# CliMA/ClimaOcean.jl

Hardware: AMD Instinct MI355X
Metric: flux-kernel surface cells/s (update_state!: JRA55 interp + similarity-theory fluxes + net fluxes) (higher is better)
Workload: dtype f64

## Files before the change

### climaocean.jl_amd/csrc/coflux_lean_kernel.hpp

```cpp
#pragma once
#include <hip/hip_runtime.h>

#include "coflux_halo_device.hpp"
#include "coflux_interp_tiles.hpp"
#include "coflux_lean.hpp"
#include "coflux_certified.hpp"
#include "coflux_solver_shared.hpp"

namespace coflux {

constexpr int LEAN_WAVES = 3;

struct LeanArgs {
    LoopParams L;
    GridDesc G;
    OceanIn O;
    Exchange E;
    FluxOut F;
    const double* g_tab;
    const DevParams* g_params;
    uint32_t* sorted;
    const int* info;
    const int* chunk_begins;
    double z_surface;
    long long mask_kind;
    double T_offset;
    unsigned long long wx_reciprocal;
    long long sort_enabled;
    IceIn I;
    NetOut N;
    SourceDesc S;
    WeightDesc Wt;
    Exchange E_next;
    long long n_chunks;
    long long tail_blocks, tail_rows, tail_cap;
    long long tail_pos;
    HaloRider H;
    long long keep_land;
};
typedef const LeanArgs __attribute__((address_space(4)))* LeanArgsPtr;

hipError_t launch_ao_lean_line(hipStream_t st, bool coare, bool fuse, bool tail, bool halo, int blocks, const LeanArgs& A);

__device__ __forceinline__ LeanArgsPtr opaque(LeanArgsPtr p) {
    asm volatile("" : "+s"(p));
    return p;
}

__device__ __forceinline__ unsigned lean_mix(unsigned idx) { return (idx * 0x9e3779b1u) ^ ((idx * 0x85ebca6bu) >> 15); }
__device__ __forceinline__ unsigned lean_sum(unsigned idx) { return idx * 0xc2b2ae35u + 0x27d4eb2fu; }

constexpr int LEAN_LIST_OFFSET = TABLE_BYTES;
constexpr int LEAN_OFFSET_BITS = 24;
constexpr unsigned LEAN_OFFSET_MASK = (1u << LEAN_OFFSET_BITS) - 1u;
static_assert((long)AO_CHUNK * AO_WET_COST < (1L << LEAN_OFFSET_BITS), "a chunk's range must fit the offset bits");
template <int BLOCK>
struct LeanGeom {
    static_assert(BLOCK == AO_BLOCK, "one workgroup geometry: 256 threads, three workgroups per CU (the 768-thread one-per-CU geometry of rounds 2-5 measured 3 % slower and was retired in round 6)");
    static constexpr int CHUNK = AO_CHUNK;
    static constexpr int WAVES = BLOCK / 64;
    static constexpr int HIST_OFFSET = LEAN_LIST_OFFSET + CHUNK * 4;
    static constexpr int CURSOR_OFFSET = HIST_OFFSET + AO_BINS * 4;
    static constexpr int COUNTERS_OFFSET = CURSOR_OFFSET + AO_BINS * 4;
    static constexpr int WAVEHASH_OFFSET = COUNTERS_OFFSET + 16;
    static constexpr int PARAMS_OFFSET = WAVEHASH_OFFSET + WAVES * 8;
    static constexpr int LDS_BYTES = PARAMS_OFFSET + (int)sizeof(DevParams);
    static_assert(PARAMS_OFFSET % 16 == 0 && LEAN_LIST_OFFSET % 1024 == 0 && (CHUNK * 4) % 1024 == 0, "LDS-DMA pieces");
};
static_assert(LeanGeom<AO_BLOCK>::LDS_BYTES <= 53760, "three narrow lean solver workgroups must fit the CU's 160 KB of LDS");

template <bool FUSE>
__device__ __forceinline__ void lean_zero_cell(const LoopParams& L, double T_offset, const GridDesc& G, LeanArgsPtr K, size_t k, int i, int j) {
    CellFluxes Z{};
    Z.Ts_ocean = -T_offset;
    Z.iterations = L.fixed ? L.maxiter : 0;
    const FluxOut F = kread(&K->F);
    store_fluxes(F, k, Z);
    if constexpr (FUSE) {
        if (i >= 0 && i < G.nx && j >= 0 && j < G.ny) {
            const NetOut N = kread(&K->N);
            store_net_cell(N, k, NetCell{});
        }
    }
}

template <bool COARE, bool FUSE, bool TAIL = false, bool CERT = false, bool LINE = false, bool HALO = false>
__device__ __forceinline__ void ao_lean_body(LeanArgsPtr K_in, int chunk_in) {
    constexpr int BLOCK = AO_BLOCK;
    using Geo = LeanGeom<BLOCK>;
    constexpr int CHUNK = Geo::CHUNK;
    LeanArgsPtr K = opaque(K_in);
    int chunk = chunk_in;
    bool wait_south = false, wait_north = false;
    if constexpr (HALO) {
        static_assert(TAIL && !CERT, "the halo riders belong to the stepping loop's exact-path launch");
        const int nh = K->H.blocks;
        if (chunk < nh) {
            extern __shared__ __attribute__((aligned(16))) char smem_h[];
            const int nf = K->H.F.n, dir = chunk / nf, f = chunk - dir * nf;
            const PeerMailbox M = kread(&K->H.M);
            const GridDesc Gh = kread(&K->G);
            peer_halo_rider(M, K->H.F.ptr[f], f, dir, K->H.rows, K->H.seq, K->H.counters, K->H.expect_sent[dir], K->H.status, Gh, BLOCK,
                            reinterpret_cast<int*>(smem_h));
            return;
        }
        chunk -= nh;
    }
    if constexpr (TAIL) {
        static_assert(BLOCK == 64 * IT_WAVES, "a tail workgroup is an interpolation workgroup");
        const int nb = (int)K->tail_blocks, ipos = (int)K->tail_pos;
        if (chunk >= ipos && chunk < ipos + nb) {
            const SourceDesc S = kread(&K->S);
            const WeightDesc Wt = kread(&K->Wt);
            const GridDesc Gt = kread(&K->G);
            const Exchange En = kread(&K->E_next);
            const int b = chunk - ipos, cap = (int)K->tail_cap, rows = (int)K->tail_rows;
            if (rows == 4) interpolate_tiles<4>(S, Wt, Gt, En, cap, b, nb);
            else if (rows == 2) interpolate_tiles<2>(S, Wt, Gt, En, cap, b, nb);
            else interpolate_tiles<1>(S, Wt, Gt, En, cap, b, nb);
            return;
        }
        if (chunk >= ipos) chunk -= nb;
    }
    if constexpr (HALO) {
        const int cs = K->H.chunk_south, cn = K->H.chunk_north, nc = (int)K->n_chunks;
        if (K->H.blocks > 0) {
            if (cs <= cn) {
                const int inner = cn - cs;
                chunk = chunk < inner ? cs + chunk : (chunk - inner < cs ? chunk - inner : cn + (chunk - inner - cs));
            }
            wait_south = K->H.wait_south != 0 && chunk < cs;
            wait_north = K->H.wait_north != 0 && chunk >= cn && chunk < nc;
        }
    }
    const LoopParams L = kread(&K->L);
    const GridDesc G = kread(&K->G);
    const double* __restrict__ g_tab = K->g_tab;
    const DevParams* __restrict__ g_params = K->g_params;
    const void* mask = K->O.mask;
    extern __shared__ __attribute__((aligned(16))) char smem[];
    double* tab = reinterpret_cast<double*>(smem);
    unsigned* list = reinterpret_cast<unsigned*>(smem + LEAN_LIST_OFFSET);
    int* hist = reinterpret_cast<int*>(smem + Geo::HIST_OFFSET);
    int* cursor = reinterpret_cast<int*>(smem + Geo::CURSOR_OFFSET);
    int* counters = reinterpret_cast<int*>(smem + Geo::COUNTERS_OFFSET);
    unsigned* wavehash = reinterpret_cast<unsigned*>(smem + Geo::WAVEHASH_OFFSET);
    DevParams* lp = reinterpret_cast<DevParams*>(smem + Geo::PARAMS_OFFSET);
    const int tid = threadIdx.x, lane = tid & 63, wave = tid >> 6;
    const int wx = G.nx + 2 * G.ring;
    const unsigned wx_rcp = (unsigned)K->wx_reciprocal;
    const bool use_static = K->sorted != nullptr;
    static_assert(sizeof(DevParams) % 16 == 0 && sizeof(DevParams) <= 1024, "the parameter block is one LDS-DMA piece");
    if (tid < (int)(sizeof(DevParams) / 16))
        __builtin_amdgcn_global_load_lds((const __attribute__((address_space(1))) void*)(reinterpret_cast<const char*>(g_params) + lane * 16),
                                         (__attribute__((address_space(3))) void*)(smem + Geo::PARAMS_OFFSET), 16, 0, 0);
    static_assert(TABLE_BYTES % 1024 == 0, "the table stage copies whole 1 KB pieces");
    {
        const char* gb = reinterpret_cast<const char*>(g_tab);
        constexpr int PIECES = TABLE_BYTES / 1024, WAVES = Geo::WAVES;
#pragma unroll
        for (int r = 0; r < (PIECES + WAVES - 1) / WAVES; ++r) {
            const int c = wave + r * WAVES;
            if (c < PIECES)
                __builtin_amdgcn_global_load_lds((const __attribute__((address_space(1))) void*)(gb + c * 1024 + lane * 16),
                                                 (__attribute__((address_space(3))) void*)(smem + c * 1024), 16, 0, 0);
        }
    }
    if (use_static) {
        const char* gl = reinterpret_cast<const char*>(K->sorted + (size_t)chunk * CHUNK);
        constexpr int PIECES = CHUNK * 4 / 1024, WAVES = Geo::WAVES;
#pragma unroll
        for (int r = 0; r < (PIECES + WAVES - 1) / WAVES; ++r) {
            const int c = wave + r * WAVES;
            if (c < PIECES)
                __builtin_amdgcn_global_load_lds((const __attribute__((address_space(1))) void*)(gl + c * 1024 + lane * 16),
                                                 (__attribute__((address_space(3))) void*)(smem + LEAN_LIST_OFFSET + c * 1024), 16, 0, 0);
        }
    }
    constexpr int LAND_UNROLL = 8;
    typedef const __attribute__((address_space(1))) unsigned* GlobalWords;
    unsigned raw_lo[LAND_UNROLL], raw_hi[LAND_UNROLL], raw_shift = 0;
    const __attribute__((address_space(4))) int* cb = (const __attribute__((address_space(4))) int*)K->chunk_begins;
    const int range_begin = cb[chunk], range_end = cb[chunk + 1];
    int listed = 0;
    unsigned want_x = 0, want_y = 0;
    if (use_static) {
        const __attribute__((address_space(4))) int* ci = (const __attribute__((address_space(4))) int*)K->info;
        listed = ci[chunk * 4];
        want_x = (unsigned)ci[chunk * 4 + 1];
        want_y = (unsigned)ci[chunk * 4 + 2];
    }
    const int mask_kind = (mask == nullptr) ? CF_MASK_NONE : (int)K->mask_kind;
    const double z_surface = K->z_surface;
    const double T_offset = K->T_offset;
    const bool keep_land = K->keep_land != 0;
    const bool sorting = !CERT && use_static && K->sort_enabled != 0;
    const int sort_windows = (int)K->sort_enabled;
    float inv_window = 0.f;
    auto lean_bin = [&](int q, int trips) -> int {
        if (sort_windows <= 1) return AO_BINS - 1 - trip_bin(trips);
        const int w = min((int)(((float)q + 0.5f) * inv_window), sort_windows - 1);
        const int bpw = AO_BINS / sort_windows, lo = bpw >= 16 ? 5 : 8;
        return w * bpw + (bpw - 1 - min(max(trips - lo, 0), bpw - 1));
    };
    {
        const unsigned long long mbase = mask_kind == CF_MASK_NONE ? (unsigned long long)g_tab : (unsigned long long)mask;
        const unsigned stride = mask_kind == CF_MASK_NONE ? 0u : (mask_kind == CF_MASK_U8 ? 1u : 8u);
        const unsigned hi_step = mask_kind == CF_MASK_BOTTOM_HEIGHT ? 4u : 0u;
#pragma unroll
        for (int n = 0; n < LAND_UNROLL; ++n) {
            const int ic = min(range_begin + tid + n * BLOCK, range_end - 1);
            const int jj = row_of(ic, wx, wx_rcp);
            const unsigned long long a = mbase + (unsigned long long)cell_index(G, ic - jj * wx - G.ring, jj - G.ring) * stride;
            raw_shift |= ((unsigned)a & 3u) << (2 * n);
            raw_lo[n] = *(GlobalWords)(a & ~3ull);
            raw_hi[n] = *(GlobalWords)((a & ~3ull) + hi_step);
        }
    }
    if (tid < 4) counters[tid] = 0;
    if (tid < AO_BINS) hist[tid] = 0;
    if constexpr (CERT) {
        if (tid < 2 * AO_BINS) hist[tid] = -1;
    }
    __builtin_amdgcn_s_waitcnt(0x0f70);
#pragma unroll
    for (int n = 0; n < LAND_UNROLL; ++n) asm volatile("" : "+v"(raw_lo[n]), "+v"(raw_hi[n]));
    unsigned hx = 0, hy = 0, land = 0;
#pragma unroll
    for (int n = 0; n < LAND_UNROLL; ++n) {
        const int idx = range_begin + tid + n * BLOCK;
        const bool w = mask_kind == CF_MASK_NONE ? true
                       : mask_kind == CF_MASK_U8 ? ((raw_lo[n] >> (8 * ((raw_shift >> (2 * n)) & 3u))) & 0xffu) != 0
                                                 : !(z_surface <= __hiloint2double((int)raw_hi[n], (int)raw_lo[n]));
        if (idx < range_end) {
            if (w) {
                hx ^= lean_mix((unsigned)idx);
                hy += lean_sum((unsigned)idx);
            } else {
                land |= 1u << n;
            }
        }
    }
    for (int idx = range_begin + tid + LAND_UNROLL * BLOCK; idx < range_end; idx += BLOCK) {
        const int jj = row_of(idx, wx, wx_rcp);
        const size_t k = cell_index(G, idx - jj * wx - G.ring, jj - G.ring);
        const bool w = mask_kind == CF_MASK_NONE ? true
                       : mask_kind == CF_MASK_U8 ? ((const uint8_t*)mask)[k] != 0 : !(z_surface <= ((const double*)mask)[k]);
        if (w) {
            hx ^= lean_mix((unsigned)idx);
            hy += lean_sum((unsigned)idx);
        } else if (!keep_land) {
            lean_zero_cell<FUSE>(L, T_offset, G, opaque(K), k, idx - jj * wx - G.ring, jj - G.ring);
        }
    }
    for (int d = 32; d; d >>= 1) {
        hx ^= (unsigned)__shfl_xor((int)hx, d);
        hy += (unsigned)__shfl_xor((int)hy, d);
    }
    if (lane == 0) {
        wavehash[2 * wave] = hx;
        wavehash[2 * wave + 1] = hy;
    }
    __syncthreads();
    if constexpr (HALO) {
        if (wait_south) peer_halo_wait(&opaque(K)->H.counters[2], K->H.expect_done[0]);
        if (wait_north) peer_halo_wait(&opaque(K)->H.counters[3], K->H.expect_done[1]);
    }
    const DevParams& P = *lp;
    bool have_list = false;
    int nwet = 0;
    if (use_static) {
        unsigned got_x = 0, got_y = 0;
#pragma unroll
        for (int w = 0; w < Geo::WAVES; ++w) {
            got_x ^= wavehash[2 * w];
            got_y += wavehash[2 * w + 1];
        }
        have_list = got_x == want_x && got_y == want_y;
        nwet = listed;
        if (sort_windows > 1 && nwet > 0)
            inv_window = 1.0f / (float)(((nwet + sort_windows * 64 - 1) / (sort_windows * 64)) * 64);
    }
    if (have_list && land && !keep_land) {
        LeanArgsPtr Kz = opaque(K);
#pragma unroll
        for (int n = 0; n < LAND_UNROLL; ++n)
            if (land & (1u << n)) {
                const int idx = range_begin + tid + n * BLOCK;
                const int jj = row_of(idx, wx, wx_rcp);
                const int i = idx - jj * wx - G.ring, j = jj - G.ring;
                lean_zero_cell<FUSE>(L, T_offset, G, Kz, cell_index(G, i, j), i, j);
            }
    }
    int begin = range_begin, end = range_end;
    for (;;) {
        if (!have_list) {
            for (int base = begin; base < end; base += BLOCK) {
                const int idx = base + tid;
                bool wet = false;
                if (idx < end) {
                    const int jj = row_of(idx, wx, wx_rcp);
                    const int i = idx - jj * wx - G.ring, j = jj - G.ring;
                    const size_t k = cell_index(G, i, j);
                    wet = cell_is_wet(P, mask, k);
                    if (!wet) lean_zero_cell<FUSE>(L, T_offset, G, opaque(K), k, i, j);
                }
                const unsigned long long m = __ballot(wet);
                int wave_base = 0;
                if (lane == 0 && m) wave_base = atomicAdd(&counters[2], __popcll(m));
                wave_base = __shfl(wave_base, 0);
                if (wet) {
                    const int p = wave_base + __popcll(m & ((1ull << lane) - 1ull));
                    if (p < CHUNK) list[p] = (unsigned)(idx - range_begin);
                }
            }
            __syncthreads();
            nwet = counters[2];
            if (nwet > CHUNK) {
                end = begin + CHUNK;
                __syncthreads();
                if (tid < 4) counters[tid] = 0;
                if constexpr (CERT) {
                    if (tid < 2 * AO_BINS) hist[tid] = -1;
                }
                __syncthreads();
                continue;
            }
        }
        auto store_result = [&](double* base, unsigned byte_off, double v) {
            if constexpr (FUSE) gstore_final(base, byte_off, v);
            else gstore(base, byte_off, v);
        };
        auto claim = [&]() {
            int st = 0;
            if (lane == 0) st = atomicAdd(&counters[0], 64);
            return __shfl(st, 0);
        };
        constexpr int QUEUE_CAP = 2 * AO_BINS;
        constexpr int QUEUE_CLOSED = 1 << 20;
        int* queue = hist;
        static_assert(Geo::CURSOR_OFFSET == Geo::HIST_OFFSET + AO_BINS * 4, "the exact-path queue spans the histogram and the cursors");
        bool straggling = false;
        int limit = nwet;
        auto position_of = [&](int st) -> int {
            const int qq = min(st + lane, limit - 1);
            if constexpr (CERT) return straggling ? queue[qq] : qq;
            return qq;
        };
        auto coords_of = [&](int st, int& ci, int& cj) -> size_t {
            const int idx = range_begin + (int)(list[position_of(st)] & LEAN_OFFSET_MASK);
            const int jj = row_of(idx, wx, wx_rcp);
            ci = idx - jj * wx - G.ring;
            cj = jj - G.ring;
            return cell_index(G, ci, cj);
        };
        auto cell_of = [&](int st) -> size_t {
            int ci, cj;
            return coords_of(st, ci, cj);
        };
        struct Raw {
            double ua, va, Ta, pa, qa, u0, u1, v0, v1, To, So;
        };
        auto request = [&](int st) {
            int ci, cj;
            const size_t k = coords_of(st, ci, cj);
            LeanArgsPtr Kb = opaque(K);
            const double* __restrict__ Ou = Kb->O.u;
            const double* __restrict__ Ov = Kb->O.v;
            const unsigned k8 = (unsigned)k * 8u;
            Raw r;
            r.u0 = gload(Ou, k8);
            r.u1 = gload(Ou, k8 + 8u);
            r.v0 = gload(Ov, k8);
            r.v1 = gload(Ov, k8 + (unsigned)G.sj * 8u);
            r.To = gload(Kb->O.T, k8);
            r.So = gload(Kb->O.S, k8);
            r.ua = gload(Kb->E.u, k8);
            r.va = gload(Kb->E.v, k8);
            r.Ta = gload(Kb->E.T, k8);
            r.pa = gload(Kb->E.p, k8);
            r.qa = gload(Kb->E.q, k8);
            return r;
        };
        int start = claim();
        Raw raw{};
        if (start < nwet) raw = request(start);
        for (;;) {
            if constexpr (CERT) {
                if (!straggling && start >= nwet) {
                    int filled = 0;
                    if (lane == 0) filled = atomicAdd(&counters[1], QUEUE_CLOSED);
                    filled = __shfl(filled, 0);
                    if (filled <= 0 || filled >= QUEUE_CLOSED) break;
                    limit = min(filled, QUEUE_CAP);
                    for (int e = lane; e < limit; e += 64)
                        while (__hip_atomic_load(&queue[e], __ATOMIC_ACQUIRE, __HIP_MEMORY_SCOPE_WORKGROUP) < 0) __builtin_amdgcn_s_sleep(1);
                    straggling = true;
                    start = 0;
                    raw = request(start);
                }
            }
            if (start >= limit) break;
            const int q = start + lane;
            const bool in_range = q < limit;
            double Mp_now = 0.0;
            const double raw_So = raw.So;
            if constexpr (CERT) {
                if (!straggling) Mp_now = gload(opaque(K)->E.Mp, (unsigned)cell_of(start) * 8u);
            }
            const LeanCell c = lean_prologue(P, L.kappa, tab, raw.ua, raw.va, raw.Ta, raw.pa, raw.qa, 0.5 * (raw.u0 + raw.u1),
                                             0.5 * (raw.v0 + raw.v1), raw.To, raw.So);
            if (in_range) store_result(opaque(K)->F.Ts, (unsigned)cell_of(start) * 8u, c.Ts - T_offset);
            CertNetSalt net_salt;
            if constexpr (CERT) {
                net_salt.Mp = (float)Mp_now;
                net_salt.floor_v = CERT_JS_FLOOR * __builtin_amdgcn_rcpf((float)raw_So * (float)P.rho_f_inv);
            }
            Scales s;
            bool finish = in_range;
            if constexpr (CERT) {
                bool exact = in_range;
                if (!straggling) {
                    const LoopParams Lc = kread(&opaque(K)->L);
                    s = mo_iterate_certified<COARE>(Lc, c, tab, in_range, exact, net_salt);
                    const unsigned long long m = __builtin_amdgcn_ballot_w64(exact);
                    const bool in_place = ((volatile int*)counters)[1] == 0 && ((volatile int*)counters)[0] >= nwet;
                    if (m && !in_place) {
                        int slot = 0;
                        if (lane == 0) slot = atomicAdd(&counters[1], __popcll(m));
                        slot = __shfl(slot, 0) + __popcll(m & ((1ull << lane) - 1ull));
                        if (exact && slot < QUEUE_CAP) {
                            __hip_atomic_store(&queue[slot], q, __ATOMIC_RELEASE, __HIP_MEMORY_SCOPE_WORKGROUP);
                            exact = false;
                            finish = false;
                        }
                    }
                }
                if (__builtin_amdgcn_ballot_w64(exact) != 0ull) {
                    const LoopParams Le = kread(&opaque(K)->L);
                    const Scales e = mo_iterate_lean<COARE, false>(Le, c, tab, exact);
                    if (exact) {
                        s = e;
                        s.it |= CERT_EXACT_FLAG;
                    }
                }
            } else {
                if constexpr (LINE) s = mo_iterate_lean_line<COARE>(L, c, tab, in_range);
                else s = mo_iterate_lean<COARE>(L, c, tab, in_range);
            }
            if (finish) {
                LeanArgsPtr Ke = opaque(K);
                const size_t k = cell_of(start);
                const CellFluxes R = lean_epilogue(c, T_offset, s);
                const FluxOut F = kread(&Ke->F);
                const unsigned k8 = (unsigned)k * 8u;
                store_result(F.Qc, k8, R.Qc);
                store_result(F.Qv, k8, R.Qv);
                store_result(F.Fv, k8, R.Fv);
                gstore(F.tx, k8, R.rho_tau_x);
                gstore(F.ty, k8, R.rho_tau_y);
                if (F.ustar) gstore_final(F.ustar, k8, R.ustar);
                if (F.tstar) gstore_final(F.tstar, k8, R.tstar);
                if (F.qstar) gstore_final(F.qstar, k8, R.qstar);
                if (F.iters) gstore_i32(F.iters, (unsigned)k * 4u, R.iterations);
                if constexpr (FUSE) {
                    const int idx = range_begin + (int)(list[position_of(start)] & LEAN_OFFSET_MASK);
                    const int jj = row_of(idx, wx, wx_rcp);
                    const int ci = idx - jj * wx - G.ring, cj = jj - G.ring;
                    if (ci >= 0 && ci < G.nx && cj >= 0 && cj < G.ny) {
                        const IceIn I = kread(&Ke->I);
                        const NetOut N = kread(&Ke->N);
                        const double Ts_ocean = (gload(Ke->O.T, k8) + P.T_offset) - T_offset;
                        const NetCell C = net_cell_local(P, P.albedo, I.conc ? gload(I.conc, k8) : 0.0, gload(Ke->O.S, k8), Ts_ocean + P.T_offset,
                                                         gload(Ke->E.Mp, k8), gload(Ke->E.Qs, k8), gload(Ke->E.Ql, k8), R.Qc, R.Qv, R.Fv,
                                                         I.Qio ? gload(I.Qio, k8) : 0.0, I.Jsio ? gload(I.Jsio, k8) : 0.0,
                                                         I.land ? gload(I.land, k8) : 0.0);
                        gstore_final(N.T, k8, C.JT);
                        gstore_final(N.S, k8, C.JS);
                        if (N.sw) gstore_final(N.sw, k8, C.sw);
                        if (N.lw_up) gstore_final(N.lw_up, k8, C.lw_up);
                        if (N.lw_down) gstore_final(N.lw_down, k8, C.lw_down);
                        if (N.sw_down) gstore_final(N.sw_down, k8, C.sw_down);
                    }
                }
                if (sorting && have_list) {
                    const int w = min(s.work, 255);
                    list[q] = (list[q] & LEAN_OFFSET_MASK) | ((unsigned)w << LEAN_OFFSET_BITS);
                    atomicAdd(&hist[lean_bin(q, w)], 1);
                }
            }
            int next;
            if constexpr (CERT) next = straggling ? start + 64 : claim();
            else next = claim();
            if (next < limit) raw = request(next);
            start = next;
        }
        if (have_list || end >= range_end) break;
        begin = end;
        end = range_end;
        __syncthreads();
        if (tid < 4) counters[tid] = 0;
        if constexpr (CERT) {
            if (tid < 2 * AO_BINS) hist[tid] = -1;
        }
        __syncthreads();
    }
    if (sorting && have_list) {
        __syncthreads();
        if (tid < AO_BINS) {
            const int v = hist[tid];
            int incl = v;
#pragma unroll
            for (int d = 1; d < 64; d <<= 1) {
                const int up = __shfl_up(incl, d);
                if (lane >= d) incl += up;
            }
            cursor[tid] = incl - v;
        }
        __syncthreads();
        uint32_t* out = opaque(K)->sorted + (size_t)chunk * CHUNK;
        constexpr int PER_THREAD = CHUNK / BLOCK;
        unsigned word[PER_THREAD];
        int at[PER_THREAD];
#pragma unroll
        for (int n = 0; n < PER_THREAD; ++n) word[n] = list[min(tid + n * BLOCK, CHUNK - 1)];
#pragma unroll
        for (int n = 0; n < PER_THREAD; ++n)
            at[n] = tid + n * BLOCK < nwet ? atomicAdd(&cursor[lean_bin(tid + n * BLOCK, (int)(word[n] >> LEAN_OFFSET_BITS))], 1) : -1;
#pragma unroll
        for (int n = 0; n < PER_THREAD; ++n)
            if (at[n] >= 0) out[at[n]] = word[n] & LEAN_OFFSET_MASK;
    }
}

}
```

### climaocean.jl_amd/csrc/coflux_solver.hip

```cpp
#include <hip/hip_runtime.h>

#include <cstring>

#include "coflux_solver_shared.hpp"
#include "coflux_lean.hpp"
#include "coflux_lean_kernel.hpp"

namespace coflux {

int wet_list_stride();
struct Geom {
    static constexpr int CHUNK = AO_CHUNK;
    static constexpr int COUNTERS_OFFSET = TABLE_DOUBLES * 8 + CHUNK * 4;
    static constexpr int PARAMS_OFFSET = COUNTERS_OFFSET + 16 + 2 * 64 * 4;
    static constexpr int LDS_BYTES = PARAMS_OFFSET + (int)sizeof(DevParams);
};
constexpr int AO_LAYER_1 = AO_CHUNK < 1024 ? AO_CHUNK : 1024, AO_LAYER_2 = AO_CHUNK < 768 ? AO_CHUNK : 768, AO_LAYER_3 = 512;
static_assert(AO_LAYER_1 <= AO_CHUNK && AO_LAYER_1 >= AO_LAYER_2 && AO_LAYER_2 >= AO_LAYER_3, "layer sizes");
static_assert(AO_BINS == 64, "Geom::PARAMS_OFFSET spells the bin count out");
static_assert(Geom::LDS_BYTES <= 53760, "three narrow solver workgroups must fit the CU's 160 KB of LDS");


constexpr int AO_MAX_ROUNDS = 8;
struct ChunkRounds {
// ... 411 lines not shown
            } else if (!keep_land) {
                SolverArgsPtr Kz = opaque(K);
                const FluxOut F = kread(&Kz->F);
                const NetOut N = kread(&Kz->N);
                zero_cell<FUSE_NET>(L, T_offset, G, F, N, k, i, j);
                        if constexpr (seaice_spec(SPEC)) ice_zero_net(opaque(K), G, k, i, j);
            }
        }
        for (int d = 32; d; d >>= 1) {
            hx ^= (unsigned)__shfl_xor((int)hx, d);
            hy ^= (unsigned)__shfl_xor((int)hy, d);
        }
        if (lane == 0) {
            atomicXor(reinterpret_cast<unsigned*>(&counters[2]), hx);
            atomicXor(reinterpret_cast<unsigned*>(&counters[3]), hy);
        }
        if (!unsorted) {
            __syncthreads();
            if (tid < 64) {
                const int v = lane < AO_BINS ? hist[lane] : 0;
                int incl = v;
#pragma unroll
                for (int d = 1; d < 64; d <<= 1) {
                    const int up = __shfl_up(incl, d);
                    if (lane >= d) incl += up;
                }
                if (lane < AO_BINS) bin_start[lane] = incl - v;
                if (lane == 63) counters[0] = incl;
            }
            __syncthreads();
#pragma unroll
            for (int n = 0; n < PER_THREAD; ++n)
                if (my_idx[n] >= 0) {
                    const int p = atomicAdd(&bin_start[AO_BINS - 1 - trip_bin(my_trip[n])], 1);
                    list[p] = ((unsigned)(tid + n * BLOCK) << AO_LIST_OFFSET_BITS) | (unsigned)(my_idx[n] - range_begin);
                }
        }
        __builtin_amdgcn_s_waitcnt(0x0f70);
        __syncthreads();
        nwet = counters[0];
        have_list = (counters[2] | counters[3]) == 0;
        if (have_list) {
            if (land && !keep_land) {
                SolverArgsPtr Kz = opaque(K);
                const FluxOut F = kread(&Kz->F);
                const NetOut N = kread(&Kz->N);
#pragma unroll
                for (int n = 0; n < LAND_UNROLL; ++n)
                    if (land & (1u << n)) {
                        const int idx = range_begin + tid + n * BLOCK;
                        const int jj = row_of(idx, wx, wx_rcp);
                        const int i = idx - jj * wx - G.ring, j = jj - G.ring;
                        zero_cell<FUSE_NET>(L, T_offset, G, F, N, cell_index(G, i, j), i, j);
                        if constexpr (seaice_spec(SPEC)) ice_zero_net(opaque(K), G, cell_index(G, i, j), i, j);
                    }
            }
        } else {
            use_static = false;
            __syncthreads();
            if (tid < 4) counters[tid] = 0;
            __syncthreads();
        }
    }
    if (!use_static) {
        __builtin_amdgcn_s_waitcnt(0x0f70);
        __syncthreads();
    }
    int begin = range_begin, end = range_end;
    for (;;) {
        if (!have_list) {
            for (int base = begin; base < end; base += BLOCK) {
                const int idx = base + tid;
                bool wet = false;
                if (idx < end) {
                    const int jj = row_of(idx, wx, wx_rcp);
                    const int i = idx - jj * wx - G.ring, j = jj - G.ring;
                    const size_t k = cell_index(G, i, j);
                    wet = cell_is_wet(P, mask, k);
                    if (!wet) {
                        SolverArgsPtr Kz = opaque(K);
                        const FluxOut F = kread(&Kz->F);
                        const NetOut N = kread(&Kz->N);
                        zero_cell<FUSE_NET>(L, T_offset, G, F, N, k, i, j);
                        if constexpr (seaice_spec(SPEC)) ice_zero_net(opaque(K), G, k, i, j);
                    }
                }
                const unsigned long long m = __ballot(wet);
                int wave_base = 0;
                if (lane == 0 && m) wave_base = atomicAdd(&counters[0], __popcll(m));
                wave_base = __shfl(wave_base, 0);
                if (wet) {
                    const int p = wave_base + __popcll(m & ((1ull << lane) - 1ull));
                    if (p < CHUNK) list[p] = (unsigned)(idx - range_begin);
                }
            }
            __builtin_amdgcn_s_waitcnt(0x0f70);
            __syncthreads();
            nwet = counters[0];
            if (nwet > CHUNK) {
                end = begin + CHUNK;
                __syncthreads();
                if (tid < 4) counters[tid] = 0;
                __syncthreads();
                continue;
            }
        }
        for (;;) {
            int start = 0;
            if (lane == 0) start = atomicAdd(&counters[1], 64);
            start = __shfl(start, 0);
            if (start >= nwet) break;
            const int q = start + lane;
            const bool in_range = q < nwet;
            const int qc = in_range ? q : nwet - 1;
            if constexpr (seaice_spec(SPEC)) {
                const IceParams Ice = kread(&K->Ice);
                IceConsts c;
                double Ts;
                bool ice_free = false;
                {
                    const int idx = range_begin + (int)(list[qc] & ((1u << AO_LIST_OFFSET_BITS) - 1u));
                    const int jj = row_of(idx, wx, wx_rcp);
                    const size_t k = cell_index(G, idx - jj * wx - G.ring, jj - G.ring);
                    SolverArgsPtr Kb = opaque(K);
                    const IceStateIn S = kread(&Kb->S);
                    const double ua = Kb->E.u[k], va = Kb->E.v[k], Ta = Kb->E.T[k], pa = Kb->E.p[k], qa = Kb->E.q[k];
                    const double inv_Ta = frcp(Ta);
                    const double lam_a = liquid_fraction_fast(P, logt, Ta);
                    const AirState A = air_state_fast(P, pa, Ta, inv_Ta, qa, lam_a, svp_equil_fast(P, logt, Ta, inv_Ta, lam_a));
                    c.rho = A.rho;
                    c.cp = A.cp_m;
                    c.qav = A.q_vap;
                    c.Ls = P.LH_s0 + (P.cp_v - P.cp_i) * (Ta - P.T_0);
                    c.Ti = Ice.T_fw - Ice.liquidus_slope * Kb->O.S[k];
                    c.hk = fmax(S.thickness[k] * Ice.inv_k, Ice.hk_min);
                    const double alb = S.albedo ? S.albedo[k] : Ice.albedo;
                    c.Qd = -(1.0 - alb) * Kb->E.Qs[k] - Ice.emissivity * Kb->E.Ql[k];
                    c.theta_a = Ta + P.g * P.h_ref * frcp(A.cp_m);
                    c.pa = pa;
                    c.du = ua;
                    c.dv = va;
                    if (P.velocity_difference == CF_VELOCITY_RELATIVE) {
                        c.du = ua - (S.u ? S.u[k] : 0.0);
                        c.dv = va - (S.v ? S.v[k] : 0.0);
                    }
                    c.dU2 = c.du * c.du + c.dv * c.dv;
                    c.dU = fsqrt(c.dU2);
                    c.dU2 = __builtin_fma(c.dU2, P.wind2_scale, P.wind2_add);
                    double alpha = P.rm.charnock;
                    if (P.rm.kind == CF_ROUGHNESS_WIND_CHARNOCK)
                        alpha = fmax(P.rm.charnock, P.rm.wind_a1 * fmin(c.dU, P.rm.wind_umax) + P.rm.wind_a2);
                    c.alpha_g = alpha * P.inv_g;
                    Ts = S.top_temperature[k] + Ice.T_offset;
                    if (Ice.ice_free_zero != 0.0 && S.concentration) ice_free = S.concentration[k] == 0.0 && S.thickness[k] == 0.0;
                }
                Scales s{0.0, 0.0, 0.0, 0, 0};
                const bool solve = in_range && !ice_free;
                if (__ballot(solve) != 0ull) {
                    bool left = false, unused = false;
                    if constexpr (seaice_lean_spec(SPEC)) {
                        const LeanIceConsts lc{c.rho, c.cp, c.qav, c.Ls, c.Ti, c.hk, c.Qd, c.theta_a, c.pa, frcp1(c.pa), frcp1(c.rho * P.R_v), c.dU2};
                        s = ice_iterate_lean<COARE, seaice_lin_spec(SPEC)>(P, L, Ice, lc, tab, solve, Ts, left);
                        if (__ballot(left) != 0ull) {
                            double Ts2 = ice_carried_skin(opaque(K), G, range_begin, list[qc], wx, wx_rcp) + Ice.T_offset;
                            const Scales s2 = ice_iterate_lean<COARE, seaice_lin_spec(SPEC), true>(P, L, Ice, lc, tab, left, Ts2, unused);
                            if (left) { s = s2; Ts = Ts2; }
                        }
                    } else {
                        s = ice_iterate<COARE, seaice_lin_spec(SPEC)>(P, L, Ice, c, tab, solve, Ts, left);
                        if (__ballot(left) != 0ull) {
                            double Ts2 = ice_carried_skin(opaque(K), G, range_begin, list[qc], wx, wx_rcp) + Ice.T_offset;
                            const Scales s2 = ice_iterate<COARE, seaice_lin_spec(SPEC), true>(P, L, Ice, c, tab, left, Ts2, unused);
                            if (left) { s = s2; Ts = Ts2; }
                        }
                    }
                }
                if (ice_free) s = Scales{0.0, 0.0, 0.0, 0, 0};
                if (in_range) {
                    SolverArgsPtr Ke = opaque(K);
                    const int idx2 = range_begin + (int)(list[qc] & ((1u << AO_LIST_OFFSET_BITS) - 1u));
                    const int jj2 = row_of(idx2, wx, wx_rcp);
                    const size_t k = cell_index(G, idx2 - jj2 * wx - G.ring, jj2 - G.ring);
                    CellFluxes R;
                    const double inv_dU = (c.dU == 0.0) ? 0.0 : frcp(c.dU);
                    const double tau = -s.us * s.us * inv_dU;
                    const double rho_u = c.rho * s.us;
                    R.Fv = -rho_u * s.qq;
                    R.Qv = R.Fv * c.Ls;
                    R.Qc = -rho_u * c.cp * s.ts;
                    R.rho_tau_x = c.rho * tau * c.du;
                    R.rho_tau_y = c.rho * tau * c.dv;
                    R.Ts_ocean = Ts - Ice.T_offset;
                    if (ice_free) R.Ts_ocean = kread(&Ke->S).top_temperature[k];
                    R.ustar = s.us;
                    R.tstar = s.ts;
                    R.qstar = s.qq;
                    R.iterations = s.it;
                    const FluxOut F = kread(&Ke->F);
                    store_fluxes(F, k, R);
                    {
                        const NetIceOut NI = kread(&Ke->NI);
                        const int ci = idx2 - jj2 * wx - G.ring, cj = jj2 - G.ring;
                        if (NI.top && ci >= 0 && ci < G.nx && cj >= 0 && cj < G.ny) {
                            const IceStateIn S2 = kread(&Ke->S);
                            double top, bottom;
                            net_sea_ice_cell(S2.albedo ? S2.albedo[k] : Ice.albedo, Ice.emissivity, Ice.eps_sigma, Ice.T_offset, Ke->E.Qs[k],
                                             Ke->E.Ql[k], R.Ts_ocean, R.Qc, R.Qv, NI.conc[k], NI.frazil ? NI.frazil[k] : 0.0,
                                             NI.interface_heat ? NI.interface_heat[k] : 0.0, top, bottom);
                            NI.top[k] = top;
                            NI.bottom[k] = bottom;
                        }
                    }
                    if (use_static && W.trip) store_hint(&W.trip[(size_t)chunk * CHUNK + (list[qc] >> AO_LIST_OFFSET_BITS)], s.work);
                }
                continue;
            }
            static_assert(SPEC != SOLVER_OCEAN_LEAN, "the ocean presets run in coflux_solver_lean.hip");
            CellConsts c;
            double So;
            {
                const int idx = range_begin + (int)(list[qc] & ((1u << AO_LIST_OFFSET_BITS) - 1u));
                const int jj = row_of(idx, wx, wx_rcp);
                const size_t k = cell_index(G, idx - jj * wx - G.ring, jj - G.ring);
                SolverArgsPtr Kb = opaque(K);
            const double* __restrict__ Ou = Kb->O.u;
            const double* __restrict__ Ov = Kb->O.v;
            const double uo = 0.5 * (Ou[k] + Ou[k + 1]);
            const double vo = 0.5 * (Ov[k] + Ov[k + (size_t)G.sj]);
                So = Kb->O.S[k];
                c = cell_prologue(P, L.min_gust, logt, Kb->E.u[k], Kb->E.v[k], Kb->E.T[k], Kb->E.p[k], Kb->E.q[k], uo, vo,
                                  Kb->O.T[k], So);
            }
            Scales s;
            if constexpr (SPEC == SOLVER_LY)
                s = ly_iterate(L, c, tab);
            else
                s = mo_iterate<COARE, SPEC>(L, c, tab, in_range);
            if (in_range) {
                SolverArgsPtr Ke = opaque(K);
                const int idx2 = range_begin + (int)(list[qc] & ((1u << AO_LIST_OFFSET_BITS) - 1u));
                const int jj2 = row_of(idx2, wx, wx_rcp);
                const int ci = idx2 - jj2 * wx - G.ring, cj = jj2 - G.ring;
                const size_t k = cell_index(G, ci, cj);
                const CellFluxes R = cell_epilogue(c, P.T_offset, s);
                {
                    const FluxOut F = kread(&Ke->F);
                    store_fluxes<FUSE_NET>(F, k, R);
                }
                if (use_static && W.trip) W.trip[(size_t)chunk * CHUNK + (list[qc] >> AO_LIST_OFFSET_BITS)] = (uint8_t)min(s.work, 255);
                if constexpr (FUSE_NET) {
                    if (ci >= 0 && ci < G.nx && cj >= 0 && cj < G.ny) {
                        const IceIn I = kread(&Ke->I);
                        const NetOut N = kread(&Ke->N);
                        store_net_cell<true>(N, k, net_cell_local(P, P.albedo, I.conc ? I.conc[k] : 0.0, So, R.Ts_ocean + P.T_offset,
                                                            Ke->E.Mp[k], Ke->E.Qs[k], Ke->E.Ql[k], R.Qc, R.Qv, R.Fv,
                                                            I.Qio ? I.Qio[k] : 0.0, I.Jsio ? I.Jsio[k] : 0.0, I.land ? I.land[k] : 0.0));
                    }
                }
            }
        }
        if (use_static || end >= range_end) break;
        begin = end;
        end = range_end;
        __syncthreads();
        if (tid < 4) counters[tid] = 0;
        __syncthreads();
    }
}

template <bool COARE, int SPEC, bool FUSE_NET, bool TAIL = false>
__global__ __launch_bounds__(AO_BLOCK, 3) void ao_flux_fast_kernel(SolverArgs unused_by_name) {
    ao_flux_fast_body<COARE, SPEC, FUSE_NET, TAIL>((SolverArgsPtr)__builtin_amdgcn_kernarg_segment_ptr(), (int)blockIdx.x);
}

struct IceOceanArgs {
    SolverArgs A;
    LeanArgs O;
    long long ocean_chunks;
    int nseg, seg_kind[8], seg_first[8], seg_count[8];
};
template <bool COARE_ICE, bool COARE_OCEAN, int ICE_SPEC>
__global__ __launch_bounds__(AO_BLOCK, 3) void ice_ocean_kernel(IceOceanArgs unused_by_name) {
    typedef const IceOceanArgs __attribute__((address_space(4)))* ArgsPtr;
    ArgsPtr K = (ArgsPtr)__builtin_amdgcn_kernarg_segment_ptr();
    asm volatile("" : "+s"(K));
    int block = (int)blockIdx.x;
    const int nch = (int)K->A.n_chunks, noc = (int)K->ocean_chunks;
    (void)noc;
    int kind = 0, idx = 0;
    {
        int rest = block;
        const int ns = K->nseg;
        for (int q = 0; q < ns; ++q) {
            const int c = K->seg_count[q];
            if (rest < c) {
                kind = K->seg_kind[q];
                idx = K->seg_first[q] + rest;
                break;
            }
            rest -= c;
        }
    }
    if (kind == 1) {
        ao_lean_body<COARE_OCEAN, true>((LeanArgsPtr)&K->O, idx);
        return;
    }
    block = kind == 2 ? nch + idx : idx;
    ao_flux_fast_body<COARE_ICE, ICE_SPEC, false, true>((SolverArgsPtr)&K->A, block);
}

__global__ void debug_eval_kernel(int fn, int n, const double* __restrict__ x, double* __restrict__ y,
                                  const double* __restrict__ g_tab) {
    extern __shared__ __attribute__((aligned(16))) char smem[];
    double* tab = reinterpret_cast<double*>(smem);
    stage_tables(tab, g_tab, threadIdx.x, blockDim.x);
    __syncthreads();
    const double* logt = tab + LOG_OFFSET;
    for (int k = blockIdx.x * blockDim.x + threadIdx.x; k < n; k += gridDim.x * blockDim.x) {
        const double v = x[k];
        double r;
        switch (fn) {
            case 0: r = flog(logt, v); break;
            case 1: r = fexp(v); break;
            case 2: r = fcbrt(v); break;
            case 3: r = fsqrt(v); break;
            case 4: r = frcp(v); break;
            case 5: r = psi_eval(tab, 0, psi_arg(v)); break;
            case 6: r = psi_eval(tab, 1, psi_arg(v)); break;
            case 7: r = __builtin_amdgcn_rcp(v); break;
            case 8: r = __builtin_amdgcn_rsq(v); break;
            case 9: {
                double q = __builtin_amdgcn_rcp(v);
                r = __builtin_fma(q, __builtin_fma(-v, q, 1.0), q);
            } break;
            default: r = 0.0;
        }
        y[k] = r;
    }
}


template <bool COARE, bool FUSE>
static void launch_ao_spec(hipStream_t st, dim3 grid, const LaunchCfg& L, const LoopParams& C, const GridDesc& G,
                           const OceanIn& O, const Exchange& E, const FluxOut& F, const IceIn& I, const NetOut& N,
                           double z_surface, long long mask_kind, double T_offset) {
    SolverArgs A{C, G, O, E, F, L.d_tables, L.d_params, WetLists{L.d_wet_pos, C.specialization == SOLVER_LY ? nullptr : L.d_trip},
                 L.d_chunk_begins, I, N, IceStateIn{}, IceParams{},
                 z_surface, mask_kind, T_offset, row_reciprocal(G.nx + 2 * G.ring)};
    A.keep_land = L.keep_land;
#define CF_LAUNCH(COARE_, SPEC_) \
    hipLaunchKernelGGL((ao_flux_fast_kernel<COARE_, SPEC_, FUSE>), grid, dim3(AO_BLOCK), Geom::LDS_BYTES, st, A)
    switch (C.specialization) {
        case SOLVER_ICE: CF_LAUNCH(COARE, SOLVER_ICE); break;
        case SOLVER_LY: CF_LAUNCH(true, SOLVER_LY); break;
        default: CF_LAUNCH(COARE, SOLVER_GENERIC);
    }
#undef CF_LAUNCH
}

hipError_t launch_ly_fluxes_with_tail(hipStream_t st, const LaunchCfg& L, const DevParams& P, const LoopParams& C, const GridDesc& G,
                                      const cf_ocean_surface* o, const cf_exchange_fields* e, const cf_interface_fluxes* f,
                                      const cf_sea_ice_fields* ice, const cf_net_ocean_fluxes* net, const double* land,
                                      const cf_atmos_source* next_src, const cf_interp_weights* w, const cf_exchange_fields* next_out,
                                      int tail_rows, int tail_blocks) {
    if (!L.d_chunk_begins || L.n_chunks <= 0 || !net || !next_src || !w || !next_out || L.interp_cap <= 0 || tail_blocks <= 0 ||
        C.specialization != SOLVER_LY)
        return hipErrorInvalidValue;
    if ((size_t)IT_WAVES * CF_JRA55_NVARS * L.interp_cap * sizeof(double) > (size_t)Geom::LDS_BYTES) return hipErrorInvalidValue;
    const IceIn I = make_ice_in(ice, land);
    const NetOut N = make_net_out(net);
    SolverArgs A{C, G, make_ocean(o), make_exchange(e), make_fluxes(f), L.d_tables, L.d_params, WetLists{L.d_wet_pos, nullptr},
                 L.d_chunk_begins, I, N, IceStateIn{}, IceParams{}, P.z_surface, P.mask_kind, P.T_offset, row_reciprocal(G.nx + 2 * G.ring)};
    A.Si = make_source(next_src);
    A.Wi = make_weights(w);
    A.E_next = make_exchange(next_out);
    A.n_chunks = L.n_chunks;
    A.tail_blocks = tail_blocks;
    A.tail_rows = tail_rows;
    A.tail_cap = L.interp_cap;
    A.keep_land = L.keep_land;
    hipLaunchKernelGGL((ao_flux_fast_kernel<true, SOLVER_LY, true, true>), dim3(L.n_chunks + tail_blocks), dim3(AO_BLOCK),
                       Geom::LDS_BYTES, st, A);
    return hipGetLastError();
}

hipError_t launch_ao_fluxes(hipStream_t st, const LaunchCfg& L, const DevParams& P, const LoopParams& C,
                            const GridDesc& G, const cf_ocean_surface* o, const cf_exchange_fields* e,
                            const cf_interface_fluxes* f, const cf_sea_ice_fields* ice, const cf_net_ocean_fluxes* net,
                            const double* land) {
    if (L.solver == CF_SOLVER_LIBM) return net ? hipErrorInvalidValue : launch_ao_fluxes_libm(st, P, G, o, e, f);
    if (C.specialization == SOLVER_OCEAN_LEAN) {
        if (!L.d_lean_info) return hipErrorInvalidValue;
        return launch_ao_fluxes_lean(st, L, P, C, G, o, e, f, ice, net, land);
    }
    OceanIn O = make_ocean(o);
    Exchange E = make_exchange(e);
    FluxOut F = make_fluxes(f);
    const IceIn I = make_ice_in(ice, land);
    const NetOut N = make_net_out(net);
    if (!L.d_chunk_begins || L.n_chunks <= 0) return hipErrorInvalidValue;
    dim3 grid(L.n_chunks);
    const bool coare = P.similarity_form == CF_SIMILARITY_COARE_LOGARITHMIC;
    if (net) {
        if (coare) launch_ao_spec<true, true>(st, grid, L, C, G, O, E, F, I, N, P.z_surface, P.mask_kind, P.T_offset);
        else launch_ao_spec<false, true>(st, grid, L, C, G, O, E, F, I, N, P.z_surface, P.mask_kind, P.T_offset);
    } else {
        if (coare) launch_ao_spec<true, false>(st, grid, L, C, G, O, E, F, I, N, P.z_surface, P.mask_kind, P.T_offset);
        else launch_ao_spec<false, false>(st, grid, L, C, G, O, E, F, I, N, P.z_surface, P.mask_kind, P.T_offset);
    }
    return hipGetLastError();
}

hipError_t launch_ai_fluxes(hipStream_t st, const LaunchCfg& L, const DevParams& P, const LoopParams& C, const IceParams& Ice,
                            const GridDesc& G, const cf_sea_ice_state* ice, const cf_ocean_surface* o,
                            const cf_exchange_fields* e, const cf_interface_fluxes* f, const double* d_tables,
                            const DevParams* d_params, uint8_t* d_trip, const AiTail* tail, const NetIceOut* net_ice) {
    if (!L.d_chunk_begins || L.n_chunks <= 0) return hipErrorInvalidValue;
    SolverArgs A{};
    A.L = C;
    A.G = G;
    A.O = make_ocean(o);
    A.E = make_exchange(e);
    A.F = make_fluxes(f);
    A.g_tab = d_tables;
    A.g_params = d_params;
    A.W = WetLists{L.d_wet_pos, d_trip};
    A.chunk_begins = L.d_chunk_begins;
    A.S = IceStateIn{ice->thickness, ice->top_temperature, ice->u, ice->v, ice->albedo, Ice.ice_free_zero != 0.0 ? ice->concentration : nullptr};
    A.Ice = Ice;
    A.z_surface = P.z_surface;
    A.mask_kind = P.mask_kind;
    A.T_offset = P.T_offset;
    A.wx_reciprocal = row_reciprocal(G.nx + 2 * G.ring);
    dim3 grid(L.n_chunks);
    const bool coare = P.similarity_form == CF_SIMILARITY_COARE_LOGARITHMIC;
    const bool lean = C.specialization == SOLVER_ICE && L.solver == CF_SOLVER_TABLES;
    const bool lin = Ice.skin_scheme == CF_SKIN_LINEARISED;
    if (net_ice) A.NI = *net_ice;
    if (tail) {
        if (!lean) return hipErrorInvalidValue;
        A.n_chunks = L.n_chunks;
        if (tail->next_out) {
            if (!tail->next_src || !tail->w || L.interp_cap <= 0 || tail->interp_blocks <= 0 ||
                (size_t)IT_WAVES * CF_JRA55_NVARS * L.interp_cap * sizeof(double) > (size_t)Geom::LDS_BYTES)
                return hipErrorInvalidValue;
            A.Si = make_source(tail->next_src);
            A.Wi = make_weights(tail->w);
            A.E_next = make_exchange(tail->next_out);
            A.tail_blocks = tail->interp_blocks;
            A.tail_rows = tail->interp_rows;
            A.tail_cap = L.interp_cap;
        }
        if (tail->stress_net) {
            if (!tail->d_ocean_params || !tail->stress_ocean || !tail->stress_fluxes) return hipErrorInvalidValue;
            A.stress_blocks = (G.nx * G.ny + 255) / 256;
            A.stress_params = tail->d_ocean_params;
            A.stress_mask = tail->stress_ocean->mask;
            A.rtx = tail->stress_fluxes->x_momentum;
            A.rty = tail->stress_fluxes->y_momentum;
            A.stress_ice = make_ice_in(tail->stress_ice, nullptr);
            A.tau_x = tail->stress_net->u;
            A.tau_y = tail->stress_net->v;
        }
        if (tail->ocean) {
            if (!tail->ocean->valid || tail->stress_net || tail->ocean->n_chunks <= 0) return hipErrorInvalidValue;
            static_assert(sizeof(LeanArgs) <= sizeof(tail->ocean->args), "OceanRider::args holds a LeanArgs");
            IceOceanArgs M{};
            M.A = A;
            memcpy(&M.O, tail->ocean->args, sizeof(LeanArgs));
            M.ocean_chunks = tail->ocean->n_chunks;
            {
                const int noc_all = tail->ocean->n_chunks, head = std::min(std::max(L.cu_count, 0), noc_all);
                M.seg_kind[0] = 1; M.seg_first[0] = 0; M.seg_count[0] = head;
                M.seg_kind[1] = 0; M.seg_first[1] = 0; M.seg_count[1] = L.n_chunks;
                M.seg_kind[2] = 1; M.seg_first[2] = head; M.seg_count[2] = noc_all - head;
                M.seg_kind[3] = 2; M.seg_first[3] = 0; M.seg_count[3] = (int)A.tail_blocks;
                M.nseg = 4;
            }
            const dim3 mgrid((unsigned)(L.n_chunks + tail->ocean->n_chunks + A.tail_blocks));
            constexpr size_t lds = (size_t)(Geom::LDS_BYTES > LeanGeom<AO_BLOCK>::LDS_BYTES ? Geom::LDS_BYTES : LeanGeom<AO_BLOCK>::LDS_BYTES);
            static_assert(lds <= 53760, "three workgroups per CU");
#define CF_IO_LAUNCH(SPEC_)                                                                                                   \
    do {                                                                                                                      \
        if (coare) {                                                                                                          \
            if (tail->ocean->coare) hipLaunchKernelGGL((ice_ocean_kernel<true, true, SPEC_>), mgrid, dim3(AO_BLOCK), lds, st, M); \
            else hipLaunchKernelGGL((ice_ocean_kernel<true, false, SPEC_>), mgrid, dim3(AO_BLOCK), lds, st, M);              \
        } else {                                                                                                              \
            if (tail->ocean->coare) hipLaunchKernelGGL((ice_ocean_kernel<false, true, SPEC_>), mgrid, dim3(AO_BLOCK), lds, st, M); \
            else hipLaunchKernelGGL((ice_ocean_kernel<false, false, SPEC_>), mgrid, dim3(AO_BLOCK), lds, st, M);             \
        }                                                                                                                     \
    } while (0)
            if (lin) CF_IO_LAUNCH(SOLVER_SEAICE_LEAN_LIN);
            else CF_IO_LAUNCH(SOLVER_SEAICE_LEAN);
#undef CF_IO_LAUNCH
            return hipGetLastError();
        }
        const dim3 tgrid((unsigned)(L.n_chunks + A.tail_blocks + A.stress_blocks));
#define CF_AI_TAIL_LAUNCH(COARE_, SPEC_) \
    hipLaunchKernelGGL((ao_flux_fast_kernel<COARE_, SPEC_, false, true>), tgrid, dim3(AO_BLOCK), Geom::LDS_BYTES, st, A)
        if (lin) { if (coare) CF_AI_TAIL_LAUNCH(true, SOLVER_SEAICE_LEAN_LIN); else CF_AI_TAIL_LAUNCH(false, SOLVER_SEAICE_LEAN_LIN); }
        else { if (coare) CF_AI_TAIL_LAUNCH(true, SOLVER_SEAICE_LEAN); else CF_AI_TAIL_LAUNCH(false, SOLVER_SEAICE_LEAN); }
#undef CF_AI_TAIL_LAUNCH
        return hipGetLastError();
    }
#define CF_AI_LAUNCH(COARE_, SPEC_) \
    hipLaunchKernelGGL((ao_flux_fast_kernel<COARE_, SPEC_, false>), grid, dim3(AO_BLOCK), Geom::LDS_BYTES, st, A)
    if (lin) {
        if (lean) { if (coare) CF_AI_LAUNCH(true, SOLVER_SEAICE_LEAN_LIN); else CF_AI_LAUNCH(false, SOLVER_SEAICE_LEAN_LIN); }
        else { if (coare) CF_AI_LAUNCH(true, SOLVER_SEAICE_LIN); else CF_AI_LAUNCH(false, SOLVER_SEAICE_LIN); }
    } else {
        if (lean) { if (coare) CF_AI_LAUNCH(true, SOLVER_SEAICE_LEAN); else CF_AI_LAUNCH(false, SOLVER_SEAICE_LEAN); }
        else { if (coare) CF_AI_LAUNCH(true, SOLVER_SEAICE); else CF_AI_LAUNCH(false, SOLVER_SEAICE); }
    }
#undef CF_AI_LAUNCH
    return hipGetLastError();
}

extern "C" int cf_debug_chunk_plan(long long total_cost, int cu_count, int forced_wet_per_chunk, int* out, int capacity) {
    ChunkRounds R{};
    plan_chunk_rounds((long)total_cost, cu_count, forced_wet_per_chunk, &R);
    if (!out || capacity < 1 + 2 * R.n) return -1;
    out[0] = R.n;
    for (int r = 0; r < R.n; ++r) {
        out[1 + 2 * r] = R.cost[r] / AO_WET_COST;
        const long span = (long)R.base[r + 1] - R.base[r];
        out[2 + 2 * r] = (int)((span + R.cost[r] - 1) / R.cost[r]);
    }
    return AO_WET_COST;
}

hipError_t launch_debug_eval(hipStream_t st, const LaunchCfg& L, int fn, int n, const double* x, double* y) {
    hipLaunchKernelGGL(debug_eval_kernel, dim3(64), dim3(256), TABLE_BYTES, st, fn, n, x, y, L.d_tables);
    return hipGetLastError();
}

}
```

Measured before the change: 10.23 billion.

## Software-pipeline lean solver: prefetch next cell and its prologue across the epilogue

In the non-certified lean path, the next cell's claim and input loads are issued before the current cell's epilogue and stores. The next cell's prologue is computed ahead of the loop body. The net-flux inputs for the current cell are also loaded early, and the coordinates come from coords_of instead of a list lookup. The aim is to hide global-memory latency behind epilogue and store work, at the cost of more live registers. The combined ocean/ice kernel explicitly opts out of this path.

Result: faster. 10.38 billion, median of 6 (+1.5%).

```diff
diff --git a/climaocean.jl_amd/csrc/coflux_lean_kernel.hpp b/climaocean.jl_amd/csrc/coflux_lean_kernel.hpp
--- a/climaocean.jl_amd/csrc/coflux_lean_kernel.hpp
+++ b/climaocean.jl_amd/csrc/coflux_lean_kernel.hpp
@@ -84,7 +84,7 @@
     }
 }
 
-template <bool COARE, bool FUSE, bool TAIL = false, bool CERT = false, bool LINE = false, bool HALO = false>
+template <bool COARE, bool FUSE, bool TAIL = false, bool CERT = false, bool LINE = false, bool HALO = false, bool BURST_BOUNDARY = true>
 __device__ __forceinline__ void ao_lean_body(LeanArgsPtr K_in, int chunk_in) {
     constexpr int BLOCK = AO_BLOCK;
     using Geo = LeanGeom<BLOCK>;
@@ -327,6 +327,7 @@
                 continue;
             }
         }
+        constexpr bool BURST = BURST_BOUNDARY && !CERT;
         auto store_result = [&](double* base, unsigned byte_off, double v) {
             if constexpr (FUSE) gstore_final(base, byte_off, v);
             else gstore(base, byte_off, v);
@@ -385,6 +386,10 @@
         int start = claim();
         Raw raw{};
         if (start < nwet) raw = request(start);
+        LeanCell ahead{};
+        if constexpr (BURST) {
+            if (start < nwet) ahead = lean_prologue(P, L.kappa, tab, raw.ua, raw.va, raw.Ta, raw.pa, raw.qa, 0.5 * (raw.u0 + raw.u1), 0.5 * (raw.v0 + raw.v1), raw.To, raw.So);
+        }
         for (;;) {
             if constexpr (CERT) {
                 if (!straggling && start >= nwet) {
@@ -408,8 +413,9 @@
             if constexpr (CERT) {
                 if (!straggling) Mp_now = gload(opaque(K)->E.Mp, (unsigned)cell_of(start) * 8u);
             }
-            const LeanCell c = lean_prologue(P, L.kappa, tab, raw.ua, raw.va, raw.Ta, raw.pa, raw.qa, 0.5 * (raw.u0 + raw.u1),
-                                             0.5 * (raw.v0 + raw.v1), raw.To, raw.So);
+            LeanCell c;
+            if constexpr (BURST) c = ahead;
+            else c = lean_prologue(P, L.kappa, tab, raw.ua, raw.va, raw.Ta, raw.pa, raw.qa, 0.5 * (raw.u0 + raw.u1), 0.5 * (raw.v0 + raw.v1), raw.To, raw.So);
             if (in_range) store_result(opaque(K)->F.Ts, (unsigned)cell_of(start) * 8u, c.Ts - T_offset);
             CertNetSalt net_salt;
             if constexpr (CERT) {
@@ -448,52 +454,125 @@
                 if constexpr (LINE) s = mo_iterate_lean_line<COARE>(L, c, tab, in_range);
                 else s = mo_iterate_lean<COARE>(L, c, tab, in_range);
             }
-            if (finish) {
-                LeanArgsPtr Ke = opaque(K);
-                const size_t k = cell_of(start);
+            if constexpr (BURST) {
+                struct NetRaw {
+                    double To, So, Mp, Qs, Ql, conc, Qio, Jsio, land;
+                };
+                auto request_net = [&](unsigned k8) {
+                    LeanArgsPtr Ke = opaque(K);
+                    NetRaw n;
+                    n.To = gload(Ke->O.T, k8);
+                    n.So = gload(Ke->O.S, k8);
+                    n.Mp = gload(Ke->E.Mp, k8);
+                    n.Qs = gload(Ke->E.Qs, k8);
+                    n.Ql = gload(Ke->E.Ql, k8);
+                    const IceIn I = kread(&Ke->I);
+                    n.conc = I.conc ? gload(I.conc, k8) : 0.0;
+                    n.Qio = I.Qio ? gload(I.Qio, k8) : 0.0;
+                    n.Jsio = I.Jsio ? gload(I.Jsio, k8) : 0.0;
+                    n.land = I.land ? gload(I.land, k8) : 0.0;
+                    return n;
+                };
+                auto net_of = [&](const NetRaw& n, const CellFluxes& R) {
+                    const double Ts_ocean = (n.To + P.T_offset) - T_offset;
+                    return net_cell_local(P, P.albedo, n.conc, n.So, Ts_ocean + P.T_offset, n.Mp, n.Qs, n.Ql, R.Qc, R.Qv, R.Fv, n.Qio, n.Jsio, n.land);
+                };
+                auto store_cell = [&](LeanArgsPtr Ke, unsigned k, const CellFluxes& R) {
+                    const FluxOut F = kread(&Ke->F);
+                    const unsigned k8 = k * 8u;
+                    store_result(F.Qc, k8, R.Qc);
+                    store_result(F.Qv, k8, R.Qv);
+                    store_result(F.Fv, k8, R.Fv);
+                    gstore(F.tx, k8, R.rho_tau_x);
+                    gstore(F.ty, k8, R.rho_tau_y);
+                    if (F.ustar) gstore_final(F.ustar, k8, R.ustar);
+                    if (F.tstar) gstore_final(F.tstar, k8, R.tstar);
+                    if (F.qstar) gstore_final(F.qstar, k8, R.qstar);
+                    if (F.iters) gstore_i32(F.iters, k * 4u, R.iterations);
+                };
+                auto store_net = [&](LeanArgsPtr Ke, unsigned k8, const NetCell& C) {
+                    const NetOut N = kread(&Ke->N);
+                    gstore_final(N.T, k8, C.JT);
+                    gstore_final(N.S, k8, C.JS);
+                    if (N.sw) gstore_final(N.sw, k8, C.sw);
+                    if (N.lw_up) gstore_final(N.lw_up, k8, C.lw_up);
+                    if (N.lw_down) gstore_final(N.lw_down, k8, C.lw_down);
+                    if (N.sw_down) gstore_final(N.sw_down, k8, C.sw_down);
+                };
+                auto note_trips = [&](int q, const Scales& s) {
+                    if (sorting && have_list) {
+                        const int w = min(s.work, 255);
+                        list[q] = (list[q] & LEAN_OFFSET_MASK) | ((unsigned)w << LEAN_OFFSET_BITS);
+                        atomicAdd(&hist[lean_bin(q, w)], 1);
+                    }
+                };
+                const int next = claim();
+                int ci, cj;
+                const unsigned k = (unsigned)coords_of(start, ci, cj);
+                NetRaw mine{};
+                if constexpr (FUSE) mine = request_net(k * 8u);
+                raw = request(next);
                 const CellFluxes R = lean_epilogue(c, T_offset, s);
-                const FluxOut F = kread(&Ke->F);
-                const unsigned k8 = (unsigned)k * 8u;
-                store_result(F.Qc, k8, R.Qc);
-                store_result(F.Qv, k8, R.Qv);
-                store_result(F.Fv, k8, R.Fv);
-                gstore(F.tx, k8, R.rho_tau_x);
-                gstore(F.ty, k8, R.rho_tau_y);
-                if (F.ustar) gstore_final(F.ustar, k8, R.ustar);
-                if (F.tstar) gstore_final(F.tstar, k8, R.tstar);
-                if (F.qstar) gstore_final(F.qstar, k8, R.qstar);
-                if (F.iters) gstore_i32(F.iters, (unsigned)k * 4u, R.iterations);
-                if constexpr (FUSE) {
-                    const int idx = range_begin + (int)(list[position_of(start)] & LEAN_OFFSET_MASK);
-                    const int jj = row_of(idx, wx, wx_rcp);
-                    const int ci = idx - jj * wx - G.ring, cj = jj - G.ring;
-                    if (ci >= 0 && ci < G.nx && cj >= 0 && cj < G.ny) {
-                        const IceIn I = kread(&Ke->I);
-                        const NetOut N = kread(&Ke->N);
-                        const double Ts_ocean = (gload(Ke->O.T, k8) + P.T_offset) - T_offset;
-                        const NetCell C = net_cell_local(P, P.albedo, I.conc ? gload(I.conc, k8) : 0.0, gload(Ke->O.S, k8), Ts_ocean + P.T_offset,
-                                                         gload(Ke->E.Mp, k8), gload(Ke->E.Qs, k8), gload(Ke->E.Ql, k8), R.Qc, R.Qv, R.Fv,
-                                                         I.Qio ? gload(I.Qio, k8) : 0.0, I.Jsio ? gload(I.Jsio, k8) : 0.0,
-                                                         I.land ? gload(I.land, k8) : 0.0);
-                        gstore_final(N.T, k8, C.JT);
-                        gstore_final(N.S, k8, C.JS);
-                        if (N.sw) gstore_final(N.sw, k8, C.sw);
-                        if (N.lw_up) gstore_final(N.lw_up, k8, C.lw_up);
-                        if (N.lw_down) gstore_final(N.lw_down, k8, C.lw_down);
-                        if (N.sw_down) gstore_final(N.sw_down, k8, C.sw_down);
+                asm volatile("" : "+v"(raw.ua), "+v"(raw.va), "+v"(raw.Ta), "+v"(raw.pa), "+v"(raw.qa), "+v"(raw.u0), "+v"(raw.u1), "+v"(raw.v0),
+                             "+v"(raw.v1), "+v"(raw.To), "+v"(raw.So));
+                if (finish) {
+                    LeanArgsPtr Ke = opaque(K);
+                    store_cell(Ke, k, R);
+                    if constexpr (FUSE) {
+                        if (ci >= 0 && ci < G.nx && cj >= 0 && cj < G.ny) store_net(Ke, k * 8u, net_of(mine, R));
                     }
-                }
-                if (sorting && have_list) {
-                    const int w = min(s.work, 255);
-                    list[q] = (list[q] & LEAN_OFFSET_MASK) | ((unsigned)w << LEAN_OFFSET_BITS);
-                    atomicAdd(&hist[lean_bin(q, w)], 1);
-                }
-            }
-            int next;
-            if constexpr (CERT) next = straggling ? start + 64 : claim();
-            else next = claim();
-            if (next < limit) raw = request(next);
-            start = next;
+                    note_trips(q, s);
+                }
+                if (next < limit) ahead = lean_prologue(P, L.kappa, tab, raw.ua, raw.va, raw.Ta, raw.pa, raw.qa, 0.5 * (raw.u0 + raw.u1), 0.5 * (raw.v0 + raw.v1), raw.To, raw.So);
+                start = next;
+            } else {
+                if (finish) {
+                    LeanArgsPtr Ke = opaque(K);
+                    const size_t k = cell_of(start);
+                    const CellFluxes R = lean_epilogue(c, T_offset, s);
+                    const FluxOut F = kread(&Ke->F);
+                    const unsigned k8 = (unsigned)k * 8u;
+                    store_result(F.Qc, k8, R.Qc);
+                    store_result(F.Qv, k8, R.Qv);
+                    store_result(F.Fv, k8, R.Fv);
+                    gstore(F.tx, k8, R.rho_tau_x);
+                    gstore(F.ty, k8, R.rho_tau_y);
+                    if (F.ustar) gstore_final(F.ustar, k8, R.ustar);
+                    if (F.tstar) gstore_final(F.tstar, k8, R.tstar);
+                    if (F.qstar) gstore_final(F.qstar, k8, R.qstar);
+                    if (F.iters) gstore_i32(F.iters, (unsigned)k * 4u, R.iterations);
+                    if constexpr (FUSE) {
+                        const int idx = range_begin + (int)(list[position_of(start)] & LEAN_OFFSET_MASK);
+                        const int jj = row_of(idx, wx, wx_rcp);
+                        const int ci = idx - jj * wx - G.ring, cj = jj - G.ring;
+                        if (ci >= 0 && ci < G.nx && cj >= 0 && cj < G.ny) {
+                            const IceIn I = kread(&Ke->I);
+                            const NetOut N = kread(&Ke->N);
+                            const double Ts_ocean = (gload(Ke->O.T, k8) + P.T_offset) - T_offset;
+                            const NetCell C = net_cell_local(P, P.albedo, I.conc ? gload(I.conc, k8) : 0.0, gload(Ke->O.S, k8), Ts_ocean + P.T_offset,
+                                                             gload(Ke->E.Mp, k8), gload(Ke->E.Qs, k8), gload(Ke->E.Ql, k8), R.Qc, R.Qv, R.Fv,
+                                                             I.Qio ? gload(I.Qio, k8) : 0.0, I.Jsio ? gload(I.Jsio, k8) : 0.0,
+                                                             I.land ? gload(I.land, k8) : 0.0);
+                            gstore_final(N.T, k8, C.JT);
+                            gstore_final(N.S, k8, C.JS);
+                            if (N.sw) gstore_final(N.sw, k8, C.sw);
+                            if (N.lw_up) gstore_final(N.lw_up, k8, C.lw_up);
+                            if (N.lw_down) gstore_final(N.lw_down, k8, C.lw_down);
+                            if (N.sw_down) gstore_final(N.sw_down, k8, C.sw_down);
+                        }
+                    }
+                    if (sorting && have_list) {
+                        const int w = min(s.work, 255);
+                        list[q] = (list[q] & LEAN_OFFSET_MASK) | ((unsigned)w << LEAN_OFFSET_BITS);
+                        atomicAdd(&hist[lean_bin(q, w)], 1);
+                    }
+                }
+                int next;
+                if constexpr (CERT) next = straggling ? start + 64 : claim();
+                else next = claim();
+                if (next < limit) raw = request(next);
+                start = next;
+            }
         }
         if (have_list || end >= range_end) break;
         begin = end;
diff --git a/climaocean.jl_amd/csrc/coflux_solver.hip b/climaocean.jl_amd/csrc/coflux_solver.hip
--- a/climaocean.jl_amd/csrc/coflux_solver.hip
+++ b/climaocean.jl_amd/csrc/coflux_solver.hip
@@ -737,7 +737,7 @@
         }
     }
     if (kind == 1) {
-        ao_lean_body<COARE_OCEAN, true>((LeanArgsPtr)&K->O, idx);
+        ao_lean_body<COARE_OCEAN, true, false, false, false, false, false>((LeanArgsPtr)&K->O, idx);
         return;
     }
     block = kind == 2 ? nch + idx : idx;
```
